# jin-s13/GKGNet

Measured on AMD Instinct MI355X. Metric: Grapher fwd+bwd images/sec, higher is better.
Workload: dtype f32; 1 GPU; BASELINE cfg2-literal: Grapher(C320,G4,k9,d1,18x18,relpos)+GrapherLabel(L80) fwd+bwd; batch_per_gpu=32, global_batch=32, C=320, G=4, HW=18x18, k=9, dilation=1, bn=local, parallelism=dp1, input_layout=nchw, launch=hipGraph replay of fwd+bwd+grad-pack, world_size=1, backend=none (single process), grad_allreduce=none (1 GPU)

## Files before the change

### gkgnet_amd/csrc/gkg_dense.hip

```cpp
#include "gkg_common.h"

namespace gkg {

template <typename OutT, bool STATS = false>
__global__ __launch_bounds__(256) void nchw_to_tm_kernel(const float* __restrict__ x, OutT* __restrict__ out,
                                                         int C, int N, const float* __restrict__ img_scale,
                                                         const float* __restrict__ add_tm = nullptr,
                                                         const float* __restrict__ y = nullptr, const float* __restrict__ mean = nullptr,
                                                         const float* __restrict__ invstd = nullptr, double* __restrict__ asums = nullptr) {
  constexpr int TS = STATS ? 4 : 1;
  __shared__ float tile[TS][32][33];
  const int b = blockIdx.z, c0 = blockIdx.y * 32, n0 = blockIdx.x * 32 * TS;
  const int tx = threadIdx.x & 31, ty = threadIdx.x >> 5;
#pragma unroll
  for (int s = 0; s < TS; ++s)
#pragma unroll
    for (int i = 0; i < 4; ++i) {
      const int ch = c0 + ty + 8 * i, n = n0 + 32 * s + tx;
      tile[s][ty + 8 * i][tx] = (ch < C && n < N) ? x[((size_t)b * C + ch) * N + n] : 0.f;
    }
  const float sc = img_scale ? img_scale[b] : 1.0f;
  float mv = 0.f, iv = 0.f, s0 = 0.f, s1 = 0.f;
  float av[TS][4], yv[TS][4];
  if constexpr (STATS) {
// ... 284 lines not shown
    const float* p = part + (size_t)q * nblk * C2 + (ln >> 2) * C + ch;
    int b = ln & 3;
    for (; b + 28 < nblk; b += 32) {
      float v[8];
#pragma unroll
      for (int u = 0; u < 8; ++u) v[u] = p[(size_t)(b + 4 * u) * C2];
#pragma unroll
      for (int u = 0; u < 8; ++u) acc += (double)v[u];
    }
    for (; b < nblk; b += 4) acc += (double)p[(size_t)b * C2];
  }
  lane_sum[ln][t] = acc;
  __syncthreads();
  if (ln != 0 || ch >= C) return;
  const double S = (lane_sum[0][t] + lane_sum[1][t]) + (lane_sum[2][t] + lane_sum[3][t]);
  const double Q = (lane_sum[4][t] + lane_sum[5][t]) + (lane_sum[6][t] + lane_sum[7][t]);
  const size_t o = (size_t)q * C + ch;
  const double ms = S / R;
  double var = Q / R - ms * ms;
  if (var < 0.0) var = 0.0;
  const double m = ms + (y_shift_row ? (double)y_shift_row[(size_t)q * R * C + ch] : 0.0);
  const float is = (float)(1.0 / sqrt(var + (double)eps));
  const float av = gamma[o] * is;
  a[o] = av;
  cs[o] = (float)((double)beta[o] - (double)av * m);
  mean[o] = (float)m;
  invstd[o] = is;
  if (running_mean) {
    const float bv = bias ? bias[o] : 0.f;
    running_mean[o] = (1.f - momentum) * running_mean[o] + momentum * ((float)m + bv);
    const double unb = R > 1 ? var * (double)R / (double)(R - 1) : var;
    running_var[o] = (1.f - momentum) * running_var[o] + momentum * (float)unb;
  }
}

__global__ void bn_finalize_kernel(const float* __restrict__ sums, const float* __restrict__ gamma,
                                   const float* __restrict__ beta, const float* __restrict__ bias,
                                   float* __restrict__ running_mean, float* __restrict__ running_var,
                                   float* __restrict__ a, float* __restrict__ cs, float* __restrict__ mean,
                                   float* __restrict__ invstd, const float* __restrict__ count, int C, float momentum,
                                   float eps, long long* __restrict__ num_batches_tracked) {
  const int ch = blockIdx.x * blockDim.x + threadIdx.x;
  if (num_batches_tracked && ch == 0 && blockIdx.y == 0) *num_batches_tracked += 1;
  if (ch >= C) return;
  const double R = (double)count[0];
  const int q = blockIdx.y;
  sums += (size_t)q * 2 * C; gamma += (size_t)q * C; beta += (size_t)q * C; a += (size_t)q * C; cs += (size_t)q * C;
  mean += (size_t)q * C; invstd += (size_t)q * C;
  if (bias) bias += (size_t)q * C;
  if (running_mean) { running_mean += (size_t)q * C; running_var += (size_t)q * C; }
  const double m = (double)sums[ch] / R;
  double var = (double)sums[C + ch] / R - m * m;
  if (var < 0.0) var = 0.0;
  const float is = (float)(1.0 / sqrt(var + (double)eps));
  const float av = gamma[ch] * is;
  a[ch] = av;
  cs[ch] = beta[ch] - av * (float)m;
  mean[ch] = (float)m;
  invstd[ch] = is;
  if (running_mean) {
    const float b = bias ? bias[ch] : 0.f;
    running_mean[ch] = (1.f - momentum) * running_mean[ch] + momentum * ((float)m + b);
    const double unb = R > 1.0 ? var * R / (R - 1.0) : var;
    running_var[ch] = (1.f - momentum) * running_var[ch] + momentum * (float)unb;
  }
}

__global__ void bn_eval_affine_kernel(const float* __restrict__ gamma, const float* __restrict__ beta,
                                      const float* __restrict__ bias, const float* __restrict__ running_mean,
                                      const float* __restrict__ running_var, float* __restrict__ a,
                                      float* __restrict__ cs, int C, float eps) {
  const int ch = blockIdx.x * blockDim.x + threadIdx.x;
  if (ch >= C) return;
  const float av = gamma[ch] / sqrtf(running_var[ch] + eps);
  a[ch] = av;
  cs[ch] = beta[ch] + av * ((bias ? bias[ch] : 0.f) - running_mean[ch]);
}

template <int ACT, typename OutT>
__global__ __launch_bounds__(256) void affine_act_kernel(const float* __restrict__ y, const float* __restrict__ a,
                                                         const float* __restrict__ cs, const float* __restrict__ res,
                                                         OutT* __restrict__ out, size_t total4, int C, int ldo,
                                                         size_t o_bstride, const float* __restrict__ row_scale,
                                                         int rows_per_scale, uint16_t* __restrict__ out2, BnDerive d,
                                                         int ochunk = 0) {
  extern __shared__ float ac_tab[];
  const int C4 = C >> 2;
  const int q = blockIdx.y;
  y += (size_t)q * total4 * 4; out += (size_t)q * o_bstride;
  if (res) res += (size_t)q * total4 * 4;
  if (d.sums) {
    const bool side = blockIdx.x == 0;
    for (int ch = threadIdx.x; ch < C; ch += 256) {
      float av, cv;
      bn_derive_channel(d, (size_t)q * C + ch, d.sums[(size_t)q * 2 * C + ch], d.sums[(size_t)q * 2 * C + C + ch], side, av, cv);
      ac_tab[ch] = av; ac_tab[C + ch] = cv;
    }
    if (side && q == 0) {
      if (threadIdx.x == 0 && d.nbt) *d.nbt += 1;
      for (size_t i = threadIdx.x; i < d.zero_doubles; i += 256) d.zero_buf[i] = 0.0;
    }
    __syncthreads();
    a = ac_tab; cs = ac_tab + C;
  } else {
    a += (size_t)q * C; cs += (size_t)q * C;
  }
  for (size_t i = (size_t)blockIdx.x * 256 + threadIdx.x; i < total4; i += (size_t)gridDim.x * 256) {
    const size_t r = i / C4;
    const int cg = (int)(i - r * C4);
    const float4 v = *reinterpret_cast<const float4*>(y + 4 * i);
    const float4 a4 = *reinterpret_cast<const float4*>(a + 4 * cg);
    const float4 c4 = *reinterpret_cast<const float4*>(cs + 4 * cg);
    float4 o;
    o.x = __builtin_fmaf(a4.x, v.x, c4.x); o.y = __builtin_fmaf(a4.y, v.y, c4.y);
    o.z = __builtin_fmaf(a4.z, v.z, c4.z); o.w = __builtin_fmaf(a4.w, v.w, c4.w);
    if (ACT == 1) { o.x = gelu_f(o.x); o.y = gelu_f(o.y); o.z = gelu_f(o.z); o.w = gelu_f(o.w); }
    if (row_scale) {
      const float sc = row_scale[r / rows_per_scale];
      o.x *= sc; o.y *= sc; o.z *= sc; o.w *= sc;
    }
    if (res) {
      const float4 rv = *reinterpret_cast<const float4*>(res + 4 * i);
      o.x += rv.x; o.y += rv.y; o.z += rv.z; o.w += rv.w;
    }
    const int oc = ochunk > 0 ? 4 * cg + (4 * cg / ochunk) * ochunk : 4 * cg;
    stf4(out + r * (size_t)ldo + oc, o);
    if (out2) stf4(out2 + r * (size_t)ldo + oc, o);
  }
}

template <int ACT>
__global__ __launch_bounds__(256) void affine_act_bf16in_kernel(const uint16_t* __restrict__ y, const float* __restrict__ a,
                                                                const float* __restrict__ cs, float* __restrict__ out32,
                                                                uint16_t* __restrict__ out16, size_t total8, int C) {
  const int C8 = C >> 3;
  for (size_t i = (size_t)blockIdx.x * 256 + threadIdx.x; i < total8; i += (size_t)gridDim.x * 256) {
    const int cg = (int)(i % C8);
    const uint4 v = *reinterpret_cast<const uint4*>(y + 8 * i);
    const uint32_t w[4] = {v.x, v.y, v.z, v.w};
    float o[8];
#pragma unroll
    for (int u = 0; u < 4; ++u) {
      o[2 * u] = __uint_as_float(w[u] << 16);
      o[2 * u + 1] = __uint_as_float(w[u] & 0xffff0000u);
    }
#pragma unroll
    for (int u = 0; u < 8; ++u) {
      o[u] = __builtin_fmaf(a[8 * cg + u], o[u], cs[8 * cg + u]);
      if (ACT == 1) o[u] = gelu_f(o[u]);
    }
    if (out32) {
      stf4(out32 + 8 * i, make_float4(o[0], o[1], o[2], o[3]));
      stf4(out32 + 8 * i + 4, make_float4(o[4], o[5], o[6], o[7]));
    }
    if (out16)
      *reinterpret_cast<uint4*>(out16 + 8 * i) = make_uint4(pack_bf16x2(o[0], o[1]), pack_bf16x2(o[2], o[3]),
                                                             pack_bf16x2(o[4], o[5]), pack_bf16x2(o[6], o[7]));
  }
}

template <int ACT>
__global__ __launch_bounds__(256) void bn_bwd_apply_d_kernel(const float* dout, const float* __restrict__ y,
                                                             const float* __restrict__ a, const float* __restrict__ cs,
                                                             const float* __restrict__ mean, const float* __restrict__ invstd,
                                                             const double* __restrict__ dsums, float* dy,
                                                             size_t total4, int C, int R, int ldg, size_t g_bstride,
                                                             float* __restrict__ dgamma, float* __restrict__ dbeta,
                                                             double* __restrict__ zero_buf, size_t zero_doubles,
                                                             const float* __restrict__ row_scale = nullptr, int rows_per_scale = 1,
                                                             const double* __restrict__ gsums = nullptr,
                                                             const float* __restrict__ count = nullptr) {
  const int C4 = C >> 2;
  const float invR = 1.0f / (count ? count[0] : (float)R);
  const int q = blockIdx.y;
  y += (size_t)q * total4 * 4; dy += (size_t)q * total4 * 4; dout += (size_t)q * g_bstride;
  a += (size_t)q * C; cs += (size_t)q * C; mean += (size_t)q * C; invstd += (size_t)q * C; dsums += (size_t)q * 2 * C;
  if (blockIdx.x == 0) {
    for (int ch = threadIdx.x; ch < C; ch += 256) {
      dbeta[(size_t)q * C + ch] = (float)dsums[ch];
      dgamma[(size_t)q * C + ch] = (float)dsums[C + ch];
    }
    if (q == 0)
      for (size_t i = threadIdx.x; i < zero_doubles; i += 256) zero_buf[i] = 0.0;
  }
  if (gsums) dsums = gsums + (size_t)q * 2 * C;
  for (size_t i = (size_t)blockIdx.x * 256 + threadIdx.x; i < total4; i += (size_t)gridDim.x * 256) {
    const size_t r = i / C4;
    const int cg = (int)(i - r * C4);
    const float4 g = *reinterpret_cast<const float4*>(dout + r * (size_t)ldg + 4 * cg);
    const float4 v = *reinterpret_cast<const float4*>(y + 4 * i);
    const float4 a4 = *reinterpret_cast<const float4*>(a + 4 * cg);
    const float4 c4 = *reinterpret_cast<const float4*>(cs + 4 * cg);
    const float4 m4 = *reinterpret_cast<const float4*>(mean + 4 * cg);
    const float4 i4 = *reinterpret_cast<const float4*>(invstd + 4 * cg);
    const double2 sa = *reinterpret_cast<const double2*>(dsums + 4 * cg), sb = *reinterpret_cast<const double2*>(dsums + 4 * cg + 2);
    const double2 qa = *reinterpret_cast<const double2*>(dsums + C + 4 * cg), qb = *reinterpret_cast<const double2*>(dsums + C + 4 * cg + 2);
    const float4 s4 = make_float4((float)sa.x, (float)sa.y, (float)sb.x, (float)sb.y);
    const float4 q4 = make_float4((float)qa.x, (float)qa.y, (float)qb.x, (float)qb.y);
    float4 dz = g;
    if (row_scale) {
      const float sc = row_scale[r / (size_t)rows_per_scale];
      dz.x *= sc; dz.y *= sc; dz.z *= sc; dz.w *= sc;
    }
    if (ACT == 1) {
      dz.x *= gelu_grad_f(__builtin_fmaf(a4.x, v.x, c4.x)); dz.y *= gelu_grad_f(__builtin_fmaf(a4.y, v.y, c4.y));
      dz.z *= gelu_grad_f(__builtin_fmaf(a4.z, v.z, c4.z)); dz.w *= gelu_grad_f(__builtin_fmaf(a4.w, v.w, c4.w));
    }
    float4 o;
    o.x = a4.x * (dz.x - s4.x * invR - ((v.x - m4.x) * i4.x) * (q4.x * invR));
    o.y = a4.y * (dz.y - s4.y * invR - ((v.y - m4.y) * i4.y) * (q4.y * invR));
// ... 86 lines not shown
#pragma unroll 4
    for (int r = r0 + rl; r < r1; r += ST_RL) {
      const float4 g = *reinterpret_cast<const float4*>(dout + (size_t)r * ldg + 4 * cgi);
      const float4 v = *reinterpret_cast<const float4*>(y + (size_t)r * C + 4 * cgi);
      float4 dz = g;
      if (row_scale) {
        const float sc = row_scale[r / rows_per_scale];
        dz.x *= sc; dz.y *= sc; dz.z *= sc; dz.w *= sc;
      }
      if (ACT == 1) {
        dz.x *= gelu_grad_f(__builtin_fmaf(a4.x, v.x, c4.x)); dz.y *= gelu_grad_f(__builtin_fmaf(a4.y, v.y, c4.y));
        dz.z *= gelu_grad_f(__builtin_fmaf(a4.z, v.z, c4.z)); dz.w *= gelu_grad_f(__builtin_fmaf(a4.w, v.w, c4.w));
      }
      *reinterpret_cast<float4*>(dy + (size_t)r * C + 4 * cgi) = make_float4(a4.x * dz.x, a4.y * dz.y, a4.z * dz.z, a4.w * dz.w);
      s[0] += (double)dz.x; s[1] += (double)dz.y; s[2] += (double)dz.z; s[3] += (double)dz.w;
      sq[0] += (double)dz.x * (double)v.x; sq[1] += (double)dz.y * (double)v.y;
      sq[2] += (double)dz.z * (double)v.z; sq[3] += (double)dz.w * (double)v.w;
    }
  }
#pragma unroll
  for (int j = 0; j < 4; ++j) { red[0][rl][4 * cg + j] = s[j]; red[1][rl][4 * cg + j] = sq[j]; }
  __syncthreads();
  if (tid < 8 * ST_CG) {
    const int which = tid >> 6, col = tid & 63;
    double acc = 0.0;
#pragma unroll
    for (int l = 0; l < ST_RL; ++l) acc += red[which][l][col];
    const int ch = blockIdx.y * 4 * ST_CG + col;
    if (ch < C) {
      if (asums) __hip_atomic_fetch_add(asums + ((size_t)q * 2 + which) * C + ch, acc, __ATOMIC_RELAXED, __HIP_MEMORY_SCOPE_AGENT);
      else part[(((size_t)q * gridDim.x + blockIdx.x) * 2 + which) * C + ch] = (float)acc;
    }
  }
}

__global__ __launch_bounds__(256) void bn_eval_bwd_finish_kernel(const double* __restrict__ dsums, const float* __restrict__ part,
                                                                 int nblk, const float* __restrict__ a,
                                                                 const float* __restrict__ running_mean,
                                                                 const float* __restrict__ running_var,
                                                                 const float* __restrict__ bias, float eps, int C,
                                                                 float* __restrict__ dgamma, float* __restrict__ dbeta,
                                                                 float* __restrict__ dbias, double* __restrict__ zero_buf,
                                                                 size_t zero_doubles) {
  const int q = blockIdx.y;
  if (blockIdx.x == 0 && q == 0)
    for (size_t i = threadIdx.x; i < zero_doubles; i += 256) zero_buf[i] = 0.0;
  const int ch = blockIdx.x * 256 + threadIdx.x;
  if (ch >= C) return;
  double S0 = 0.0, S1 = 0.0;
  if (dsums) {
    S0 = dsums[(size_t)q * 2 * C + ch];
    S1 = dsums[(size_t)q * 2 * C + C + ch];
  } else {
    const float* p = part + (size_t)q * nblk * 2 * C + ch;
    for (int b = 0; b < nblk; ++b) { S0 += (double)p[(size_t)b * 2 * C]; S1 += (double)p[(size_t)b * 2 * C + C]; }
  }
  const size_t o = (size_t)q * C + ch;
  if (dbeta) dbeta[o] = (float)S0;
  if (dgamma) {
    const double sh = (bias ? (double)bias[o] : 0.0) - (double)running_mean[o];
    dgamma[o] = (float)((S1 + sh * S0) / sqrt((double)running_var[o] + (double)eps));
  }
  if (dbias) dbias[o] = (float)((double)a[o] * S0);
}

}

using namespace gkg;

static int stats_tiles(int C) { return ((C >> 2) + ST_CG - 1) / ST_CG; }

static int stats_blocks(int R, int C, int nb, int* rows_per_block) {
  const int cols = stats_tiles(C) * nb;
  int nblk = (768 + cols - 1) / cols;
  const int cap = cols >= 4 ? 128 : 256;
  if (nblk > cap) nblk = cap;
  const int by_rows = (R + ST_RL - 1) / ST_RL;
  if (nblk > by_rows) nblk = by_rows;
  if (nblk < 1) nblk = 1;
  *rows_per_block = (R + nblk - 1) / nblk;
  return (R + *rows_per_block - 1) / *rows_per_block;
}

static bool bad_c(int C) { return C <= 0 || (C & 3) != 0 || C > 4096; }

extern "C" size_t gkg_bn_workspace_bytes(int R, int C, int nb) {
  if (R <= 0 || bad_c(C) || nb <= 0) return 0;
  int rpb;
  const int nblk = stats_blocks(R, C, nb, &rpb);
  return (size_t)nb * (nblk + 1) * 2 * C * sizeof(float);
}

extern "C" int gkg_nchw_to_tm(const float* x, void* out, int B, int C, int N, int out_dtype, const float* img_scale,
                              void* stream) {
  if (!x || !out) return gkg_fail(GKG_ERR_NULL, "gkg_nchw_to_tm: null pointer");
  if (B <= 0 || C <= 0 || N <= 0 || B > 65535) return gkg_fail(GKG_ERR_SHAPE, "gkg_nchw_to_tm: bad sizes");
  if (out_dtype != GKG_F32 && out_dtype != GKG_BF16) return gkg_fail(GKG_ERR_UNSUPPORTED, "gkg_nchw_to_tm: out_dtype is GKG_F32 or GKG_BF16");
  dim3 grid((N + 31) / 32, (C + 31) / 32, B);
  if (out_dtype == GKG_BF16) hipLaunchKernelGGL(nchw_to_tm_kernel<uint16_t>, grid, dim3(256), 0, (hipStream_t)stream, x, (uint16_t*)out, C, N, img_scale);
  else hipLaunchKernelGGL(nchw_to_tm_kernel<float>, grid, dim3(256), 0, (hipStream_t)stream, x, (float*)out, C, N, img_scale);
  hipError_t e = hipGetLastError();
  return e == hipSuccess ? 0 : gkg_fail_hip(e, "nchw_to_tm_kernel");
}

extern "C" int gkg_nchw_to_tm_add(const float* x, const float* add_tm, float* out, int B, int C, int N, void* stream) {
  if (!x || !add_tm || !out) return gkg_fail(GKG_ERR_NULL, "gkg_nchw_to_tm_add: null pointer");
  if (B <= 0 || C <= 0 || N <= 0 || B > 65535) return gkg_fail(GKG_ERR_SHAPE, "gkg_nchw_to_tm_add: bad sizes");
  dim3 grid((N + 31) / 32, (C + 31) / 32, B);
  hipLaunchKernelGGL(nchw_to_tm_kernel<float>, grid, dim3(256), 0, (hipStream_t)stream, x, out, C, N, (const float*)nullptr, add_tm);
  hipError_t e = hipGetLastError();
  return e == hipSuccess ? 0 : gkg_fail_hip(e, "nchw_to_tm_kernel (add)");
}

extern "C" int gkg_nchw_to_tm_add_bnstats(const float* x, const float* add_tm, float* out, const float* y, const float* mean,
                                          const float* invstd, double* sums, int B, int C, int N, void* stream) {
  if (!x || !out || !y || !mean || !invstd || !sums) return gkg_fail(GKG_ERR_NULL, "gkg_nchw_to_tm_add_bnstats: null pointer");
  if (B <= 0 || C <= 0 || N <= 0 || B > 65535) return gkg_fail(GKG_ERR_SHAPE, "gkg_nchw_to_tm_add_bnstats: bad sizes");
  dim3 grid((N + 127) / 128, (C + 31) / 32, B);
  hipLaunchKernelGGL((nchw_to_tm_kernel<float, true>), grid, dim3(256), 0, (hipStream_t)stream, x, out, C, N, (const float*)nullptr, add_tm,
                     y, mean, invstd, sums);
  hipError_t e = hipGetLastError();
  return e == hipSuccess ? 0 : gkg_fail_hip(e, "nchw_to_tm_kernel (add + BN backward statistics)");
}

extern "C" int gkg_tm_affine_to_nchw_dual(const float* y, const float* a, const float* c, const float* res_tm, float* out,
                                          float* out_tm, int B, int C, int N, void* stream) {
  if (!y || !out || !res_tm || !out_tm || ((a == nullptr) != (c == nullptr))) return gkg_fail(GKG_ERR_NULL, "gkg_tm_affine_to_nchw_dual: null pointer");
  if (B <= 0 || C <= 0 || N <= 0 || B > 65535) return gkg_fail(GKG_ERR_SHAPE, "gkg_tm_affine_to_nchw_dual: bad sizes");
  dim3 grid((N + 31) / 32, (C + 31) / 32, B);
  hipLaunchKernelGGL(tm_affine_to_nchw_kernel, grid, dim3(256), 0, (hipStream_t)stream, y, a, c, (const float*)nullptr, out, C, N,
                     (const float*)nullptr, BnDerive{}, res_tm, out_tm);
  hipError_t e = hipGetLastError();
  return e == hipSuccess ? 0 : gkg_fail_hip(e, "tm_affine_to_nchw_kernel (dual)");
}

extern "C" int gkg_tm_affine_to_nchw(const float* y, const float* a, const float* c, const float* res, float* out,
                                     int B, int C, int N, const float* img_scale, void* stream) {
  if (!y || !out || ((a == nullptr) != (c == nullptr))) return gkg_fail(GKG_ERR_NULL, "gkg_tm_affine_to_nchw: null pointer");
  if (B <= 0 || C <= 0 || N <= 0 || B > 65535) return gkg_fail(GKG_ERR_SHAPE, "gkg_tm_affine_to_nchw: bad sizes");
  dim3 grid((N + 31) / 32, (C + 31) / 32, B);
  hipLaunchKernelGGL(tm_affine_to_nchw_kernel, grid, dim3(256), 0, (hipStream_t)stream, y, a, c, res, out, C, N, img_scale, BnDerive{});
  hipError_t e = hipGetLastError();
  return e == hipSuccess ? 0 : gkg_fail_hip(e, "tm_affine_to_nchw_kernel");
}

extern "C" int gkg_bn_train_stats(const float* y, const float* gamma, const float* beta, const float* bias,
                                  float* running_mean, float* running_var, float* a, float* c, float* mean,
                                  float* invstd, int R, int C, int nb, float momentum, float eps,
                                  long long* num_batches_tracked, void* workspace, size_t workspace_bytes, void* stream) {
  if (!y || !gamma || !beta || !a || !c || !mean || !invstd || !workspace)
    return gkg_fail(GKG_ERR_NULL, "gkg_bn_train_stats: null pointer");
  if (R <= 0 || bad_c(C) || nb <= 0 || nb > 64) return gkg_fail(GKG_ERR_SHAPE, "gkg_bn_train_stats: need R > 0, C % 4 == 0, C <= 4096, 1 <= nb <= 64");
  if ((running_mean == nullptr) != (running_var == nullptr)) return gkg_fail(GKG_ERR_NULL, "gkg_bn_train_stats: running stats come in pairs");
  int rpb;
  const int nblk = stats_blocks(R, C, nb, &rpb);
  if (workspace_bytes < (size_t)nb * (nblk + 1) * 2 * C * sizeof(float))
    return gkg_fail(GKG_ERR_WORKSPACE, "gkg_bn_train_stats: workspace too small (gkg_bn_workspace_bytes)");
  hipStream_t st = (hipStream_t)stream;
  float* part = (float*)workspace;
  float* sums = part + (size_t)nb * nblk * 2 * C;
  hipLaunchKernelGGL(col_stats_kernel<true>, dim3(nblk, stats_tiles(C), nb), dim3(256), 0, st, y, part, R, C, rpb);
  hipLaunchKernelGGL(reduce_finalize_kernel, dim3((C + 31) / 32, nb), dim3(256), 0, st, part, nblk, gamma, beta, bias,
                     running_mean, running_var, a, c, mean, invstd, R, C, momentum, eps, num_batches_tracked, y);
  hipError_t e = hipGetLastError();
  return e == hipSuccess ? 0 : gkg_fail_hip(e, "bn_train_stats");
}

extern "C" int gkg_bn_eval_affine(const float* gamma, const float* beta, const float* bias, const float* running_mean,
                                  const float* running_var, float* a, float* c, int C, float eps, void* stream) {
  if (!gamma || !beta || !running_mean || !running_var || !a || !c) return gkg_fail(GKG_ERR_NULL, "gkg_bn_eval_affine: null pointer");
  if (C <= 0) return gkg_fail(GKG_ERR_SHAPE, "gkg_bn_eval_affine: bad C");
  hipLaunchKernelGGL(bn_eval_affine_kernel, dim3((C + 255) / 256), dim3(256), 0, (hipStream_t)stream, gamma, beta, bias,
                     running_mean, running_var, a, c, C, eps);
  hipError_t e = hipGetLastError();
  return e == hipSuccess ? 0 : gkg_fail_hip(e, "bn_eval_affine_kernel");
}

extern "C" int gkg_avgpool_tm(const float* x, int ldx, int xchunk, float* out, int B, int H, int W, int C, int r, void* stream) {
  if (!x || !out) return gkg_fail(GKG_ERR_NULL, "gkg_avgpool_tm: null pointer");
  if (ldx == 0) ldx = C;
  if (B <= 0 || H <= 0 || W <= 0 || bad_c(C) || r <= 0 || H / r <= 0 || W / r <= 0 || ldx < C || (ldx & 3) || xchunk < 0 || (xchunk & 3) ||
      (xchunk > 0 && (C % xchunk || ldx < 2 * C)) || ((size_t)x & 15) || ((size_t)out & 15))
    return gkg_fail(GKG_ERR_SHAPE, "gkg_avgpool_tm: bad sizes (C % 4 == 0, r <= H, W; 16-byte aligned rows)");
  const size_t total4 = (size_t)B * (H / r) * (W / r) * (C >> 2);
  if ((total4 + 255) / 256 > 0x7fffffffull) return gkg_fail(GKG_ERR_UNSUPPORTED, "gkg_avgpool_tm: too large for one launch");
  hipLaunchKernelGGL(avgpool_tm_kernel, dim3((unsigned)((total4 + 255) / 256)), dim3(256), 0, (hipStream_t)stream, x, out, H, W, C, r, ldx,
                     xchunk, total4);
  hipError_t e = hipGetLastError();
  return e == hipSuccess ? 0 : gkg_fail_hip(e, "avgpool_tm_kernel");
}

extern "C" int gkg_affine_act(const float* y, const float* a, const float* c, const float* res, void* out, int R, int C,
                              int nb, int ldo, size_t out_bstride, int ochunk, int act, int out_dtype, const float* row_scale,
                              int rows_per_scale, void* stream) {
  if (row_scale && rows_per_scale <= 0) return gkg_fail(GKG_ERR_SHAPE, "gkg_affine_act: rows_per_scale must be positive");
  if (ochunk < 0 || (ochunk & 3) || (ochunk > 0 && (C % ochunk || ldo < 2 * C)))
    return gkg_fail(GKG_ERR_SHAPE, "gkg_affine_act: ochunk must be a multiple of 4 dividing C, with ldo >= 2 C");
  if (!y || !a || !c || !out) return gkg_fail(GKG_ERR_NULL, "gkg_affine_act: null pointer");
  if (R <= 0 || bad_c(C) || nb <= 0 || nb > 64 || ldo < C || (ldo & 3) || (out_bstride & 3) || (act != 0 && act != 1))
    return gkg_fail(GKG_ERR_SHAPE, "gkg_affine_act: bad sizes");
  if (out_dtype != GKG_F32 && out_dtype != GKG_BF16) return gkg_fail(GKG_ERR_UNSUPPORTED, "gkg_affine_act: out_dtype is GKG_F32 or GKG_BF16");
  const size_t total4 = (size_t)R * (C >> 2);
  const int blocks = (int)((total4 + 255) / 256 > 2048 ? 2048 : (total4 + 255) / 256);
  const dim3 grid(blocks, nb);
  hipStream_t st = (hipStream_t)stream;
  if (out_dtype == GKG_BF16) {
    uint16_t* o = (uint16_t*)out;
    if (act == 1) hipLaunchKernelGGL((affine_act_kernel<1, uint16_t>), grid, dim3(256), 0, st, y, a, c, res, o, total4, C, ldo, out_bstride, row_scale, rows_per_scale, (uint16_t*)nullptr, BnDerive{}, ochunk);
    else hipLaunchKernelGGL((affine_act_kernel<0, uint16_t>), grid, dim3(256), 0, st, y, a, c, res, o, total4, C, ldo, out_bstride, row_scale, rows_per_scale, (uint16_t*)nullptr, BnDerive{}, ochunk);
  } else {
    float* o = (float*)out;
    if (act == 1) hipLaunchKernelGGL((affine_act_kernel<1, float>), grid, dim3(256), 0, st, y, a, c, res, o, total4, C, ldo, out_bstride, row_scale, rows_per_scale, (uint16_t*)nullptr, BnDerive{}, ochunk);
    else hipLaunchKernelGGL((affine_act_kernel<0, float>), grid, dim3(256), 0, st, y, a, c, res, o, total4, C, ldo, out_bstride, row_scale, rows_per_scale, (uint16_t*)nullptr, BnDerive{}, ochunk);
  }
  hipError_t e = hipGetLastError();
  return e == hipSuccess ? 0 : gkg_fail_hip(e, "affine_act_kernel");
}

extern "C" int gkg_affine_act_bf16in(const void* y_bf16, const float* a, const float* c, float* out_f32, void* out_bf16, int R,
                                     int C, int act, void* stream) {
  if (!y_bf16 || !a || !c || (!out_f32 && !out_bf16)) return gkg_fail(GKG_ERR_NULL, "gkg_affine_act_bf16in: null pointer");
  if (R <= 0 || C <= 0 || (C & 7) || (act != 0 && act != 1)) return gkg_fail(GKG_ERR_SHAPE, "gkg_affine_act_bf16in: bad sizes (C % 8 == 0)");
  const size_t total8 = (size_t)R * (C >> 3);
  const int blocks = (int)((total8 + 255) / 256 > 4096 ? 4096 : (total8 + 255) / 256);
  hipStream_t st = (hipStream_t)stream;
  if (act == 1) hipLaunchKernelGGL((affine_act_bf16in_kernel<1>), dim3(blocks), dim3(256), 0, st, (const uint16_t*)y_bf16, a, c, out_f32, (uint16_t*)out_bf16, total8, C);
  else hipLaunchKernelGGL((affine_act_bf16in_kernel<0>), dim3(blocks), dim3(256), 0, st, (const uint16_t*)y_bf16, a, c, out_f32, (uint16_t*)out_bf16, total8, C);
  hipError_t e = hipGetLastError();
  return e == hipSuccess ? 0 : gkg_fail_hip(e, "affine_act_bf16in_kernel");
}

extern "C" int gkg_affine_act_dual(const float* y, const float* a, const float* c, const float* res, float* out_f32,
                                   void* out_bf16, int R, int C, int act, const float* row_scale, int rows_per_scale,
                                   void* stream) {
  if (row_scale && rows_per_scale <= 0) return gkg_fail(GKG_ERR_SHAPE, "gkg_affine_act_dual: rows_per_scale must be positive");
  if (!y || !a || !c || !out_f32 || !out_bf16) return gkg_fail(GKG_ERR_NULL, "gkg_affine_act_dual: null pointer");
  if (R <= 0 || bad_c(C) || (act != 0 && act != 1)) return gkg_fail(GKG_ERR_SHAPE, "gkg_affine_act_dual: bad sizes");
  const size_t total4 = (size_t)R * (C >> 2);
  const int blocks = (int)((total4 + 255) / 256 > 2048 ? 2048 : (total4 + 255) / 256);
  hipStream_t st = (hipStream_t)stream;
  if (act == 1) hipLaunchKernelGGL((affine_act_kernel<1, float>), dim3(blocks, 1), dim3(256), 0, st, y, a, c, res, out_f32, total4, C, C, (size_t)0, row_scale, rows_per_scale, (uint16_t*)out_bf16, BnDerive{});
  else hipLaunchKernelGGL((affine_act_kernel<0, float>), dim3(blocks, 1), dim3(256), 0, st, y, a, c, res, out_f32, total4, C, C, (size_t)0, row_scale, rows_per_scale, (uint16_t*)out_bf16, BnDerive{});
  hipError_t e = hipGetLastError();
  return e == hipSuccess ? 0 : gkg_fail_hip(e, "affine_act_kernel (dual)");
}

extern "C" int gkg_bn_bwd(const float* dout, const float* y, const float* a, const float* c, const float* mean,
                          const float* invstd, float* dy, float* dgamma, float* dbeta, int R, int C, int nb, int ldg,
                          size_t dout_bstride, int act, void* workspace, size_t workspace_bytes, void* stream) {
  if (!dout || !y || !a || !c || !mean || !invstd || !dy || !dgamma || !dbeta || !workspace)
    return gkg_fail(GKG_ERR_NULL, "gkg_bn_bwd: null pointer");
  if (R <= 0 || bad_c(C) || nb <= 0 || nb > 64 || ldg < C || (ldg & 3) || (dout_bstride & 3) || (act != 0 && act != 1))
    return gkg_fail(GKG_ERR_SHAPE, "gkg_bn_bwd: bad sizes");
  int rpb;
  const int nblk = stats_blocks(R, C, nb, &rpb);
  if (workspace_bytes < (size_t)nb * (nblk + 1) * 2 * C * sizeof(float)) return gkg_fail(GKG_ERR_WORKSPACE, "gkg_bn_bwd: workspace too small");
  hipStream_t st = (hipStream_t)stream;
  float* part = (float*)workspace;
  float* sums = part + (size_t)nb * nblk * 2 * C;
  if (act == 1) hipLaunchKernelGGL((bn_bwd_stats_kernel<1>), dim3(nblk, stats_tiles(C), nb), dim3(256), 0, st, dout, y, a, c, mean, invstd, part, R, C, rpb, ldg, dout_bstride, (float*)nullptr);
  else hipLaunchKernelGGL((bn_bwd_stats_kernel<0>), dim3(nblk, stats_tiles(C), nb), dim3(256), 0, st, dout, y, a, c, mean, invstd, part, R, C, rpb, ldg, dout_bstride, (float*)nullptr);
  hipLaunchKernelGGL(reduce_partials_kernel, dim3((2 * C + 31) / 32, nb), dim3(256), 0, st, part, sums, nblk, 2 * C, dbeta, dgamma);
  const size_t total4 = (size_t)R * (C >> 2);
  const int blocks = (int)((total4 + 255) / 256 > 2048 ? 2048 : (total4 + 255) / 256);
  if (act == 1) hipLaunchKernelGGL((bn_bwd_apply_kernel<1>), dim3(blocks, nb), dim3(256), 0, st, dout, y, a, c, mean, invstd, sums, dy, total4, C, R, ldg, dout_bstride, (const float*)nullptr);
  else hipLaunchKernelGGL((bn_bwd_apply_kernel<0>), dim3(blocks, nb), dim3(256), 0, st, dout, y, a, c, mean, invstd, sums, dy, total4, C, R, ldg, dout_bstride, (const float*)nullptr);
  hipError_t e = hipGetLastError();
  return e == hipSuccess ? 0 : gkg_fail_hip(e, "bn_bwd");
}

static int bn_bwd_atomic_impl(const float* dout, const float* y, const float* a, const float* c, const float* mean,
                              const float* invstd, float* dy, float* dgamma, float* dbeta, int R, int C, int nb, int ldg,
                              size_t dout_bstride, int act, double* sums, double* zero_buf, size_t zero_doubles, void* stream,
                              bool stats_pass, const float* row_scale = nullptr, int rows_per_scale = 1, bool apply_pass = true,
                              const double* gsums = nullptr, const float* count = nullptr);

extern "C" int gkg_bn_bwd_atomic(const float* dout, const float* y, const float* a, const float* c, const float* mean,
                                 const float* invstd, float* dy, float* dgamma, float* dbeta, int R, int C, int nb, int ldg,
                                 size_t dout_bstride, int act, double* sums, double* zero_buf, size_t zero_doubles, void* stream) {
  if (!dout || !y || !a || !c || !mean || !invstd || !dy || !dgamma || !dbeta || !sums)
    return gkg_fail(GKG_ERR_NULL, "gkg_bn_bwd_atomic: null pointer");
  if (R <= 0 || bad_c(C) || nb <= 0 || nb > 64 || ldg < C || (ldg & 3) || (dout_bstride & 3) || (act != 0 && act != 1) ||
      (zero_doubles && !zero_buf))
    return gkg_fail(GKG_ERR_SHAPE, "gkg_bn_bwd_atomic: bad sizes");
  return bn_bwd_atomic_impl(dout, y, a, c, mean, invstd, dy, dgamma, dbeta, R, C, nb, ldg, dout_bstride, act, sums, zero_buf,
                            zero_doubles, stream, true);
}

extern "C" int gkg_bn_bwd_atomic_scaled(const float* dout, const float* y, const float* a, const float* c, const float* mean,
                                        const float* invstd, float* dy, float* dgamma, float* dbeta, int R, int C, int nb,
                                        int ldg, size_t dout_bstride, int act, double* sums, double* zero_buf,
                                        size_t zero_doubles, const float* row_scale, int rows_per_scale, void* stream) {
  if (!dout || !y || !a || !c || !mean || !invstd || !dy || !dgamma || !dbeta || !sums || !row_scale)
    return gkg_fail(GKG_ERR_NULL, "gkg_bn_bwd_atomic_scaled: null pointer");
  if (R <= 0 || bad_c(C) || nb <= 0 || nb > 64 || ldg < C || (ldg & 3) || (dout_bstride & 3) || (act != 0 && act != 1) ||
      (zero_doubles && !zero_buf) || rows_per_scale <= 0)
    return gkg_fail(GKG_ERR_SHAPE, "gkg_bn_bwd_atomic_scaled: bad sizes");
  return bn_bwd_atomic_impl(dout, y, a, c, mean, invstd, dy, dgamma, dbeta, R, C, nb, ldg, dout_bstride, act, sums, zero_buf,
                            zero_doubles, stream, true, row_scale, rows_per_scale);
}

extern "C" int gkg_bn_bwd_apply_from_sums(const float* dout, const float* y, const float* a, const float* c, const float* mean,
                                          const float* invstd, float* dy, float* dgamma, float* dbeta, int R, int C, int nb,
                                          int ldg, size_t dout_bstride, int act, const double* sums, double* zero_buf,
                                          size_t zero_doubles, void* stream) {
  if (!dout || !y || !a || !c || !mean || !invstd || !dy || !dgamma || !dbeta || !sums)
    return gkg_fail(GKG_ERR_NULL, "gkg_bn_bwd_apply_from_sums: null pointer");
  if (R <= 0 || bad_c(C) || nb <= 0 || nb > 64 || ldg < C || (ldg & 3) || (dout_bstride & 3) || (act != 0 && act != 1) ||
      (zero_doubles && !zero_buf))
    return gkg_fail(GKG_ERR_SHAPE, "gkg_bn_bwd_apply_from_sums: bad sizes");
  return bn_bwd_atomic_impl(dout, y, a, c, mean, invstd, dy, dgamma, dbeta, R, C, nb, ldg, dout_bstride, act,
                            const_cast<double*>(sums), zero_buf, zero_doubles, stream, false);
}

extern "C" int gkg_bn_eval_bwd(const float* dout, const float* y, const float* a, const float* c, float* dy, int R, int C, int nb,
                               int ldg, size_t dout_bstride, int act, const float* row_scale, int rows_per_scale,
                               const float* running_mean, const float* running_var, const float* bias, float eps, float* dgamma,
                               float* dbeta, float* dbias, double* sums, double* zero_buf, size_t zero_doubles, void* workspace,
                               size_t workspace_bytes, void* stream) {
  if (!dout || !y || !a || !c || !dy) return gkg_fail(GKG_ERR_NULL, "gkg_bn_eval_bwd: null pointer");
  if (R <= 0 || bad_c(C) || nb <= 0 || nb > 64 || ldg < C || (ldg & 3) || (dout_bstride & 3) || (act != 0 && act != 1) ||
      (zero_doubles && !zero_buf) || (row_scale && rows_per_scale <= 0))
    return gkg_fail(GKG_ERR_SHAPE, "gkg_bn_eval_bwd: bad sizes");
  const bool want = dgamma || dbeta || dbias;
  if (dgamma && (!running_mean || !running_var)) return gkg_fail(GKG_ERR_NULL, "gkg_bn_eval_bwd: dgamma needs the running statistics");
// ... 15 lines not shown
  else { if (act == 1) GKG_EVAL_BWD(1, false); else GKG_EVAL_BWD(0, false); }
#undef GKG_EVAL_BWD
  if (want)
    hipLaunchKernelGGL(bn_eval_bwd_finish_kernel, dim3((C + 255) / 256, nb), dim3(256), 0, st, (const double*)sums, (const float*)part, nblk,
                       a, running_mean, running_var, bias, eps, C, dgamma, dbeta, dbias, zero_buf, zero_doubles);
  hipError_t e = hipGetLastError();
  return e == hipSuccess ? 0 : gkg_fail_hip(e, "bn_eval_bwd");
}


static int bn_bwd_atomic_impl(const float* dout, const float* y, const float* a, const float* c, const float* mean,
                              const float* invstd, float* dy, float* dgamma, float* dbeta, int R, int C, int nb, int ldg,
                              size_t dout_bstride, int act, double* sums, double* zero_buf, size_t zero_doubles, void* stream,
                              bool stats_pass, const float* row_scale, int rows_per_scale, bool apply_pass, const double* gsums,
                              const float* count) {
  int rpb;
  const int nblk = stats_blocks(R, C, nb, &rpb);
  hipStream_t st = (hipStream_t)stream;
  if (stats_pass) {
    if (act == 1) hipLaunchKernelGGL((bn_bwd_stats_kernel<1>), dim3(nblk, stats_tiles(C), nb), dim3(256), 0, st, dout, y, a, c, mean, invstd, (float*)nullptr, R, C, rpb, ldg, dout_bstride, (float*)nullptr, sums, row_scale, rows_per_scale);
    else hipLaunchKernelGGL((bn_bwd_stats_kernel<0>), dim3(nblk, stats_tiles(C), nb), dim3(256), 0, st, dout, y, a, c, mean, invstd, (float*)nullptr, R, C, rpb, ldg, dout_bstride, (float*)nullptr, sums, row_scale, rows_per_scale);
  }
  if (apply_pass) {
    const size_t total4 = (size_t)R * (C >> 2);
    const int blocks = (int)((total4 + 255) / 256 > 2048 ? 2048 : (total4 + 255) / 256);
    if (act == 1) hipLaunchKernelGGL((bn_bwd_apply_d_kernel<1>), dim3(blocks, nb), dim3(256), 0, st, dout, y, a, c, mean, invstd, sums, dy, total4, C, R, ldg, dout_bstride, dgamma, dbeta, zero_buf, zero_doubles, row_scale, rows_per_scale, gsums, count);
    else hipLaunchKernelGGL((bn_bwd_apply_d_kernel<0>), dim3(blocks, nb), dim3(256), 0, st, dout, y, a, c, mean, invstd, sums, dy, total4, C, R, ldg, dout_bstride, dgamma, dbeta, zero_buf, zero_doubles, row_scale, rows_per_scale, gsums, count);
  }
  hipError_t e = hipGetLastError();
  return e == hipSuccess ? 0 : gkg_fail_hip(e, "bn_bwd_atomic");
}

extern "C" int gkg_bn_bwd_stats_f64(const float* dout, const float* y, const float* a, const float* c, const float* mean,
                                    const float* invstd, int R, int C, int nb, int ldg, size_t dout_bstride, int act, double* sums,
                                    const float* row_scale, int rows_per_scale, void* stream) {
  if (!dout || !y || !a || !c || !mean || !invstd || !sums) return gkg_fail(GKG_ERR_NULL, "gkg_bn_bwd_stats_f64: null pointer");
  if (R <= 0 || bad_c(C) || nb <= 0 || nb > 64 || ldg < C || (ldg & 3) || (dout_bstride & 3) || (act != 0 && act != 1) ||
      (row_scale && rows_per_scale <= 0))
    return gkg_fail(GKG_ERR_SHAPE, "gkg_bn_bwd_stats_f64: bad sizes");
  return bn_bwd_atomic_impl(dout, y, a, c, mean, invstd, nullptr, nullptr, nullptr, R, C, nb, ldg, dout_bstride, act, sums, nullptr, 0,
                            stream, true, row_scale, row_scale ? rows_per_scale : 1, false);
}

extern "C" int gkg_bn_bwd_apply_sync(const float* dout, const float* y, const float* a, const float* c, const float* mean,
                                     const float* invstd, float* dy, float* dgamma, float* dbeta, int R, int C, int nb, int ldg,
                                     size_t dout_bstride, int act, const double* sums_local, const double* sums_global,
                                     const float* count, double* zero_buf, size_t zero_doubles, const float* row_scale,
                                     int rows_per_scale, void* stream) {
  if (!dout || !y || !a || !c || !mean || !invstd || !dy || !dgamma || !dbeta || !sums_local || !sums_global || !count)
    return gkg_fail(GKG_ERR_NULL, "gkg_bn_bwd_apply_sync: null pointer");
  if (R <= 0 || bad_c(C) || nb <= 0 || nb > 64 || ldg < C || (ldg & 3) || (dout_bstride & 3) || (act != 0 && act != 1) ||
      (zero_doubles && !zero_buf) || (row_scale && rows_per_scale <= 0) || (((size_t)sums_local | (size_t)sums_global) & 15))
    return gkg_fail(GKG_ERR_SHAPE, "gkg_bn_bwd_apply_sync: bad sizes");
  return bn_bwd_atomic_impl(dout, y, a, c, mean, invstd, dy, dgamma, dbeta, R, C, nb, ldg, dout_bstride, act,
                            const_cast<double*>(sums_local), zero_buf, zero_doubles, stream, false, row_scale,
                            row_scale ? rows_per_scale : 1, true, sums_global, count);
}

static int bn_apply_train_impl(const float* y, const double* sums, const float* gamma, const float* beta, const float* bias,
                               float* running_mean, float* running_var, long long* num_batches_tracked, float* a, float* c,
                               float* mean, float* invstd, const float* res, float* out, int R, int C, int nb, int ldo,
                               size_t out_bstride, int ochunk, int act, int nchw_B, const float* row_scale, int rows_per_scale,
                               float momentum, float eps, double* zero_buf, size_t zero_doubles, void* stream,
                               const double* count, float* count_out) {
  if (!y || !sums || !gamma || !beta || !a || !c || !mean || !invstd || !out)
    return gkg_fail(GKG_ERR_NULL, "gkg_bn_apply_train: null pointer");
  if ((running_mean == nullptr) != (running_var == nullptr)) return gkg_fail(GKG_ERR_NULL, "gkg_bn_apply_train: running stats come in pairs");
  if (R <= 0 || bad_c(C) || nb <= 0 || nb > 64 || (act != 0 && act != 1) || (zero_doubles && !zero_buf) || nchw_B < 0)
    return gkg_fail(GKG_ERR_SHAPE, "gkg_bn_apply_train: bad sizes");
  BnDerive d{sums, gamma, beta, bias, running_mean, running_var, num_batches_tracked, a, c, mean, invstd, R, momentum, eps,
             zero_buf, zero_doubles, count, count_out};
  hipStream_t st = (hipStream_t)stream;
  if (nchw_B > 0) {
    if (nb != 1 || act != 0 || R % nchw_B) return gkg_fail(GKG_ERR_SHAPE, "gkg_bn_apply_train: channel-major output needs nb == 1, act == 0, R % B == 0");
    const int N = R / nchw_B;
    dim3 grid((N + 31) / 32, (C + 31) / 32, nchw_B);
    hipLaunchKernelGGL(tm_affine_to_nchw_kernel, grid, dim3(256), 0, st, y, (const float*)nullptr, (const float*)nullptr, res, out, C, N,
                       row_scale, d);
  } else {
    if (row_scale && rows_per_scale <= 0) return gkg_fail(GKG_ERR_SHAPE, "gkg_bn_apply_train: rows_per_scale must be positive");
    if (ldo < C || (ldo & 3) || (out_bstride & 3)) return gkg_fail(GKG_ERR_SHAPE, "gkg_bn_apply_train: bad output pitch");
    if (ochunk < 0 || (ochunk & 3) || (ochunk > 0 && (C % ochunk || ldo < 2 * C)))
      return gkg_fail(GKG_ERR_SHAPE, "gkg_bn_apply_train: ochunk must be a multiple of 4 dividing C, with ldo >= 2 C");
    const size_t total4 = (size_t)R * (C >> 2);
    const int blocks = (int)((total4 + 255) / 256 > 2048 ? 2048 : (total4 + 255) / 256);
    const dim3 grid(blocks, nb);
    const size_t lds = (size_t)2 * C * sizeof(float);
    if (act == 1) hipLaunchKernelGGL((affine_act_kernel<1, float>), grid, dim3(256), lds, st, y, (const float*)nullptr, (const float*)nullptr, res, out, total4, C, ldo, out_bstride, row_scale, rows_per_scale, (uint16_t*)nullptr, d, ochunk);
    else hipLaunchKernelGGL((affine_act_kernel<0, float>), grid, dim3(256), lds, st, y, (const float*)nullptr, (const float*)nullptr, res, out, total4, C, ldo, out_bstride, row_scale, rows_per_scale, (uint16_t*)nullptr, d, ochunk);
  }
  hipError_t e = hipGetLastError();
  return e == hipSuccess ? 0 : gkg_fail_hip(e, "bn_apply_train");
}

extern "C" int gkg_bn_apply_train(const float* y, const double* sums, const float* gamma, const float* beta, const float* bias,
                                  float* running_mean, float* running_var, long long* num_batches_tracked, float* a, float* c,
                                  float* mean, float* invstd, const float* res, float* out, int R, int C, int nb, int ldo,
                                  size_t out_bstride, int ochunk, int act, int nchw_B, const float* row_scale, int rows_per_scale,
                                  float momentum, float eps, double* zero_buf, size_t zero_doubles, void* stream) {
  return bn_apply_train_impl(y, sums, gamma, beta, bias, running_mean, running_var, num_batches_tracked, a, c, mean, invstd, res, out,
                             R, C, nb, ldo, out_bstride, ochunk, act, nchw_B, row_scale, rows_per_scale, momentum, eps, zero_buf,
                             zero_doubles, stream, nullptr, nullptr);
}

extern "C" int gkg_bn_apply_train_sync(const float* y, const double* sums, const float* gamma, const float* beta, const float* bias,
                                       float* running_mean, float* running_var, long long* num_batches_tracked, float* a, float* c,
                                       float* mean, float* invstd, const float* res, float* out, int R, int C, int nb, int ldo,
                                       size_t out_bstride, int ochunk, int act, int nchw_B, const float* row_scale,
                                       int rows_per_scale, float momentum, float eps, double* zero_buf, size_t zero_doubles,
                                       const double* count, float* count_out, void* stream) {
  if (!count) return gkg_fail(GKG_ERR_NULL, "gkg_bn_apply_train_sync: null count");
  return bn_apply_train_impl(y, sums, gamma, beta, bias, running_mean, running_var, num_batches_tracked, a, c, mean, invstd, res, out,
                             R, C, nb, ldo, out_bstride, ochunk, act, nchw_B, row_scale, rows_per_scale, momentum, eps, zero_buf,
                             zero_doubles, stream, count, count_out);
}

static int bn_apply_train_dual_impl(const float* y, const double* sums, const float* gamma, const float* beta, const float* bias,
                                    float* running_mean, float* running_var, long long* num_batches_tracked, float* a,
                                    float* c, float* mean, float* invstd, const float* res_tm, float* out, float* out_tm,
                                    int B, int C, int N, float momentum, float eps, double* zero_buf, size_t zero_doubles,
                                    void* stream, const double* count, float* count_out) {
  if (!y || !sums || !gamma || !beta || !a || !c || !mean || !invstd || !out || !res_tm || !out_tm)
    return gkg_fail(GKG_ERR_NULL, "gkg_bn_apply_train_dual: null pointer");
  if ((running_mean == nullptr) != (running_var == nullptr)) return gkg_fail(GKG_ERR_NULL, "gkg_bn_apply_train_dual: running stats come in pairs");
  if (B <= 0 || B > 65535 || N <= 0 || bad_c(C) || (zero_doubles && !zero_buf)) return gkg_fail(GKG_ERR_SHAPE, "gkg_bn_apply_train_dual: bad sizes");
  BnDerive d{sums, gamma, beta, bias, running_mean, running_var, num_batches_tracked, a, c, mean, invstd, B * N, momentum, eps,
             zero_buf, zero_doubles, count, count_out};
  dim3 grid((N + 31) / 32, (C + 31) / 32, B);
  hipLaunchKernelGGL(tm_affine_to_nchw_kernel, grid, dim3(256), 0, (hipStream_t)stream, y, (const float*)nullptr, (const float*)nullptr,
                     (const float*)nullptr, out, C, N, (const float*)nullptr, d, res_tm, out_tm);
  hipError_t e = hipGetLastError();
  return e == hipSuccess ? 0 : gkg_fail_hip(e, "bn_apply_train (dual)");
}

extern "C" int gkg_bn_apply_train_dual(const float* y, const double* sums, const float* gamma, const float* beta, const float* bias,
                                       float* running_mean, float* running_var, long long* num_batches_tracked, float* a,
                                       float* c, float* mean, float* invstd, const float* res_tm, float* out, float* out_tm,
                                       int B, int C, int N, float momentum, float eps, double* zero_buf, size_t zero_doubles,
                                       void* stream) {
  return bn_apply_train_dual_impl(y, sums, gamma, beta, bias, running_mean, running_var, num_batches_tracked, a, c, mean, invstd,
                                  res_tm, out, out_tm, B, C, N, momentum, eps, zero_buf, zero_doubles, stream, nullptr, nullptr);
}

extern "C" int gkg_bn_apply_train_dual_sync(const float* y, const double* sums, const float* gamma, const float* beta,
                                            const float* bias, float* running_mean, float* running_var,
                                            long long* num_batches_tracked, float* a, float* c, float* mean, float* invstd,
                                            const float* res_tm, float* out, float* out_tm, int B, int C, int N, float momentum,
                                            float eps, double* zero_buf, size_t zero_doubles, const double* count, float* count_out,
                                            void* stream) {
  if (!count) return gkg_fail(GKG_ERR_NULL, "gkg_bn_apply_train_dual_sync: null count");
  return bn_apply_train_dual_impl(y, sums, gamma, beta, bias, running_mean, running_var, num_batches_tracked, a, c, mean, invstd,
                                  res_tm, out, out_tm, B, C, N, momentum, eps, zero_buf, zero_doubles, stream, count, count_out);
}

extern "C" int gkg_bn_stats_sums(const float* y, float* sums, int R, int C, int nb, void* workspace,
                                 size_t workspace_bytes, void* stream) {
  if (!y || !sums || !workspace) return gkg_fail(GKG_ERR_NULL, "gkg_bn_stats_sums: null pointer");
  if (R <= 0 || bad_c(C) || nb <= 0 || nb > 64) return gkg_fail(GKG_ERR_SHAPE, "gkg_bn_stats_sums: bad sizes");
  int rpb;
  const int nblk = stats_blocks(R, C, nb, &rpb);
  if (workspace_bytes < (size_t)nb * (nblk + 1) * 2 * C * sizeof(float))
    return gkg_fail(GKG_ERR_WORKSPACE, "gkg_bn_stats_sums: workspace too small (gkg_bn_workspace_bytes)");
  hipStream_t st = (hipStream_t)stream;
  float* part = (float*)workspace;
  hipLaunchKernelGGL(col_stats_kernel<false>, dim3(nblk, stats_tiles(C), nb), dim3(256), 0, st, y, part, R, C, rpb);
  hipLaunchKernelGGL(reduce_partials_kernel, dim3((2 * C + 31) / 32, nb), dim3(256), 0, st, part, sums, nblk, 2 * C,
                     (float*)nullptr, (float*)nullptr);
  hipError_t e = hipGetLastError();
  return e == hipSuccess ? 0 : gkg_fail_hip(e, "bn_stats_sums");
}

extern "C" int gkg_bn_finalize(const float* sums, const float* count, const float* gamma, const float* beta,
// ... 47 lines not shown
```

Baseline: 41220 images/s.

## Tile BN train-apply by channel slice so each block derives only its channels

Replaces the grid-stride BN apply used in training with a 2D-tiled kernel. Each block now covers a column slice of channels and a row range, so it derives scale and shift only for its own channels instead of every block recomputing all C channels from double sums. Loads of the first rows are issued before the derive step, and rows are prefetched in groups of four. This adds more template variants and a heuristic for tile and block counts.

```diff
diff --git a/gkgnet_amd/csrc/gkg_dense.hip b/gkgnet_amd/csrc/gkg_dense.hip
--- a/gkgnet_amd/csrc/gkg_dense.hip
+++ b/gkgnet_amd/csrc/gkg_dense.hip
@@ -390,29 +390,12 @@
                                                          const float* __restrict__ cs, const float* __restrict__ res,
                                                          OutT* __restrict__ out, size_t total4, int C, int ldo,
                                                          size_t o_bstride, const float* __restrict__ row_scale,
-                                                         int rows_per_scale, uint16_t* __restrict__ out2, BnDerive d,
-                                                         int ochunk = 0) {
-  extern __shared__ float ac_tab[];
+                                                         int rows_per_scale, uint16_t* __restrict__ out2, int ochunk = 0) {
   const int C4 = C >> 2;
   const int q = blockIdx.y;
   y += (size_t)q * total4 * 4; out += (size_t)q * o_bstride;
   if (res) res += (size_t)q * total4 * 4;
-  if (d.sums) {
-    const bool side = blockIdx.x == 0;
-    for (int ch = threadIdx.x; ch < C; ch += 256) {
-      float av, cv;
-      bn_derive_channel(d, (size_t)q * C + ch, d.sums[(size_t)q * 2 * C + ch], d.sums[(size_t)q * 2 * C + C + ch], side, av, cv);
-      ac_tab[ch] = av; ac_tab[C + ch] = cv;
-    }
-    if (side && q == 0) {
-      if (threadIdx.x == 0 && d.nbt) *d.nbt += 1;
-      for (size_t i = threadIdx.x; i < d.zero_doubles; i += 256) d.zero_buf[i] = 0.0;
-    }
-    __syncthreads();
-    a = ac_tab; cs = ac_tab + C;
-  } else {
-    a += (size_t)q * C; cs += (size_t)q * C;
-  }
+  a += (size_t)q * C; cs += (size_t)q * C;
   for (size_t i = (size_t)blockIdx.x * 256 + threadIdx.x; i < total4; i += (size_t)gridDim.x * 256) {
     const size_t r = i / C4;
     const int cg = (int)(i - r * C4);
@@ -434,6 +417,74 @@
     const int oc = ochunk > 0 ? 4 * cg + (4 * cg / ochunk) * ochunk : 4 * cg;
     stf4(out + r * (size_t)ldo + oc, o);
     if (out2) stf4(out2 + r * (size_t)ldo + oc, o);
+  }
+}
+
+constexpr int AP_PF = 4;
+template <int ACT, bool RES>
+__global__ __launch_bounds__(256) void bn_apply_tiled_kernel(const float* __restrict__ y, const float* __restrict__ res,
+                                                             float* __restrict__ out, int R, int C, int ldo, size_t o_bstride,
+                                                             const float* __restrict__ row_scale, int rows_per_scale, BnDerive d,
+                                                             int ochunk, int tile4, int rows_per_block) {
+  __shared__ float ac_tab[2][256];
+  const int tid = threadIdx.x;
+  const int q = blockIdx.z;
+  const int C4 = C >> 2;
+  const int RL = 256 / tile4;
+  const int rl = tid / tile4;
+  const int cg = tid - rl * tile4;
+  const int cgi = blockIdx.y * tile4 + cg;
+  const int r1 = (int)min((long long)R, ((long long)blockIdx.x + 1) * rows_per_block);
+  y += (size_t)q * R * C + 4 * min(cgi, C4 - 1); out += (size_t)q * o_bstride;
+  if (RES) res += (size_t)q * R * C + 4 * min(cgi, C4 - 1);
+  int r = (rl < RL && cgi < C4) ? (int)blockIdx.x * rows_per_block + rl : r1;
+  const int chd = blockIdx.y * 4 * tile4 + tid;
+  const bool derive = tid < 4 * tile4 && chd < C;
+  double S = 0.0, Q = 0.0;
+  if (derive) { S = d.sums[(size_t)q * 2 * C + chd]; Q = d.sums[(size_t)q * 2 * C + C + chd]; }
+  float4 v[AP_PF], rv[AP_PF];
+  float sc[AP_PF];
+  auto request = [&]() __attribute__((always_inline)) {
+#pragma unroll
+    for (int u = 0; u < AP_PF; ++u) {
+      const int ru = min(r + u * RL, r1 - 1);
+      v[u] = *reinterpret_cast<const float4*>(y + (size_t)ru * C);
+      if (RES) rv[u] = *reinterpret_cast<const float4*>(res + (size_t)ru * C);
+      if (row_scale) sc[u] = row_scale[ru / rows_per_scale];
+    }
+  };
+  request();
+  if (derive) {
+    float av, cv;
+    bn_derive_channel(d, (size_t)q * C + chd, S, Q, blockIdx.x == 0, av, cv);
+    ac_tab[0][tid] = av; ac_tab[1][tid] = cv;
+  }
+  if (blockIdx.x == 0 && blockIdx.y == 0 && q == 0) {
+    if (tid == 0 && d.nbt) *d.nbt += 1;
+    for (size_t i = tid; i < d.zero_doubles; i += 256) d.zero_buf[i] = 0.0;
+  }
+  __syncthreads();
+  if (r >= r1) return;
+  const float4 a4 = *reinterpret_cast<const float4*>(&ac_tab[0][4 * cg]);
+  const float4 c4 = *reinterpret_cast<const float4*>(&ac_tab[1][4 * cg]);
+  out += ochunk > 0 ? 4 * cgi + (4 * cgi / ochunk) * ochunk : 4 * cgi;
+  for (;;) {
+#pragma unroll
+    for (int u = 0; u < AP_PF; ++u) {
+      const int ru = r + u * RL;
+      if (ru < r1) {
+        float4 o;
+        o.x = __builtin_fmaf(a4.x, v[u].x, c4.x); o.y = __builtin_fmaf(a4.y, v[u].y, c4.y);
+        o.z = __builtin_fmaf(a4.z, v[u].z, c4.z); o.w = __builtin_fmaf(a4.w, v[u].w, c4.w);
+        if (ACT == 1) { o.x = gelu_f(o.x); o.y = gelu_f(o.y); o.z = gelu_f(o.z); o.w = gelu_f(o.w); }
+        if (row_scale) { o.x *= sc[u]; o.y *= sc[u]; o.z *= sc[u]; o.w *= sc[u]; }
+        if (RES) { o.x += rv[u].x; o.y += rv[u].y; o.z += rv[u].z; o.w += rv[u].w; }
+        stf4(out + (size_t)ru * ldo, o);
+      }
+    }
+    r += AP_PF * RL;
+    if (r >= r1) break;
+    request();
   }
 }
 
@@ -686,6 +737,19 @@
   return (R + *rows_per_block - 1) / *rows_per_block;
 }
 
+static int apply_blocks(int R, int C, int nb, int act, int* tile4, int* rows_per_block) {
+  const int C4 = C >> 2;
+  const int tiles = (C4 + 63) / 64;
+  *tile4 = (C4 & 15) == 0 ? 16 : (C4 + tiles - 1) / tiles;
+  const int min_rows = (act == 1 ? 1 : AP_PF) * (256 / *tile4);
+  const int cols = ((C4 + *tile4 - 1) / *tile4) * nb;
+  long long nblk = (1024 + cols - 1) / cols;
+  const long long by_rows = ((long long)R + min_rows - 1) / min_rows;
+  if (nblk > by_rows) nblk = by_rows;
+  *rows_per_block = (int)((R + nblk - 1) / nblk);
+  return (int)((R + (long long)*rows_per_block - 1) / *rows_per_block);
+}
+
 static bool bad_c(int C) { return C <= 0 || (C & 3) != 0 || C > 4096; }
 
 extern "C" size_t gkg_bn_workspace_bytes(int R, int C, int nb) {
@@ -810,12 +874,12 @@
   hipStream_t st = (hipStream_t)stream;
   if (out_dtype == GKG_BF16) {
     uint16_t* o = (uint16_t*)out;
-    if (act == 1) hipLaunchKernelGGL((affine_act_kernel<1, uint16_t>), grid, dim3(256), 0, st, y, a, c, res, o, total4, C, ldo, out_bstride, row_scale, rows_per_scale, (uint16_t*)nullptr, BnDerive{}, ochunk);
-    else hipLaunchKernelGGL((affine_act_kernel<0, uint16_t>), grid, dim3(256), 0, st, y, a, c, res, o, total4, C, ldo, out_bstride, row_scale, rows_per_scale, (uint16_t*)nullptr, BnDerive{}, ochunk);
+    if (act == 1) hipLaunchKernelGGL((affine_act_kernel<1, uint16_t>), grid, dim3(256), 0, st, y, a, c, res, o, total4, C, ldo, out_bstride, row_scale, rows_per_scale, (uint16_t*)nullptr, ochunk);
+    else hipLaunchKernelGGL((affine_act_kernel<0, uint16_t>), grid, dim3(256), 0, st, y, a, c, res, o, total4, C, ldo, out_bstride, row_scale, rows_per_scale, (uint16_t*)nullptr, ochunk);
   } else {
     float* o = (float*)out;
-    if (act == 1) hipLaunchKernelGGL((affine_act_kernel<1, float>), grid, dim3(256), 0, st, y, a, c, res, o, total4, C, ldo, out_bstride, row_scale, rows_per_scale, (uint16_t*)nullptr, BnDerive{}, ochunk);
-    else hipLaunchKernelGGL((affine_act_kernel<0, float>), grid, dim3(256), 0, st, y, a, c, res, o, total4, C, ldo, out_bstride, row_scale, rows_per_scale, (uint16_t*)nullptr, BnDerive{}, ochunk);
+    if (act == 1) hipLaunchKernelGGL((affine_act_kernel<1, float>), grid, dim3(256), 0, st, y, a, c, res, o, total4, C, ldo, out_bstride, row_scale, rows_per_scale, (uint16_t*)nullptr, ochunk);
+    else hipLaunchKernelGGL((affine_act_kernel<0, float>), grid, dim3(256), 0, st, y, a, c, res, o, total4, C, ldo, out_bstride, row_scale, rows_per_scale, (uint16_t*)nullptr, ochunk);
   }
   hipError_t e = hipGetLastError();
   return e == hipSuccess ? 0 : gkg_fail_hip(e, "affine_act_kernel");
@@ -843,8 +907,8 @@
   const size_t total4 = (size_t)R * (C >> 2);
   const int blocks = (int)((total4 + 255) / 256 > 2048 ? 2048 : (total4 + 255) / 256);
   hipStream_t st = (hipStream_t)stream;
-  if (act == 1) hipLaunchKernelGGL((affine_act_kernel<1, float>), dim3(blocks, 1), dim3(256), 0, st, y, a, c, res, out_f32, total4, C, C, (size_t)0, row_scale, rows_per_scale, (uint16_t*)out_bf16, BnDerive{});
-  else hipLaunchKernelGGL((affine_act_kernel<0, float>), dim3(blocks, 1), dim3(256), 0, st, y, a, c, res, out_f32, total4, C, C, (size_t)0, row_scale, rows_per_scale, (uint16_t*)out_bf16, BnDerive{});
+  if (act == 1) hipLaunchKernelGGL((affine_act_kernel<1, float>), dim3(blocks, 1), dim3(256), 0, st, y, a, c, res, out_f32, total4, C, C, (size_t)0, row_scale, rows_per_scale, (uint16_t*)out_bf16);
+  else hipLaunchKernelGGL((affine_act_kernel<0, float>), dim3(blocks, 1), dim3(256), 0, st, y, a, c, res, out_f32, total4, C, C, (size_t)0, row_scale, rows_per_scale, (uint16_t*)out_bf16);
   hipError_t e = hipGetLastError();
   return e == hipSuccess ? 0 : gkg_fail_hip(e, "affine_act_kernel (dual)");
 }
@@ -1026,12 +1090,12 @@
     if (ldo < C || (ldo & 3) || (out_bstride & 3)) return gkg_fail(GKG_ERR_SHAPE, "gkg_bn_apply_train: bad output pitch");
     if (ochunk < 0 || (ochunk & 3) || (ochunk > 0 && (C % ochunk || ldo < 2 * C)))
       return gkg_fail(GKG_ERR_SHAPE, "gkg_bn_apply_train: ochunk must be a multiple of 4 dividing C, with ldo >= 2 C");
-    const size_t total4 = (size_t)R * (C >> 2);
-    const int blocks = (int)((total4 + 255) / 256 > 2048 ? 2048 : (total4 + 255) / 256);
-    const dim3 grid(blocks, nb);
-    const size_t lds = (size_t)2 * C * sizeof(float);
-    if (act == 1) hipLaunchKernelGGL((affine_act_kernel<1, float>), grid, dim3(256), lds, st, y, (const float*)nullptr, (const float*)nullptr, res, out, total4, C, ldo, out_bstride, row_scale, rows_per_scale, (uint16_t*)nullptr, d, ochunk);
-    else hipLaunchKernelGGL((affine_act_kernel<0, float>), grid, dim3(256), lds, st, y, (const float*)nullptr, (const float*)nullptr, res, out, total4, C, ldo, out_bstride, row_scale, rows_per_scale, (uint16_t*)nullptr, d, ochunk);
+    if (R > 0x7fffffff - 4 * 256 * AP_PF) return gkg_fail(GKG_ERR_UNSUPPORTED, "gkg_bn_apply_train: too many rows for one launch");
+    int tile4, rpb;
+    const dim3 grid(apply_blocks(R, C, nb, act, &tile4, &rpb), ((C >> 2) + tile4 - 1) / tile4, nb);
+    auto kern = act == 1 ? (res ? bn_apply_tiled_kernel<1, true> : bn_apply_tiled_kernel<1, false>)
+                         : (res ? bn_apply_tiled_kernel<0, true> : bn_apply_tiled_kernel<0, false>);
+    hipLaunchKernelGGL(kern, grid, dim3(256), 0, st, y, res, out, R, C, ldo, out_bstride, row_scale, rows_per_scale, d, ochunk, tile4, rpb);
   }
   hipError_t e = hipGetLastError();
   return e == hipSuccess ? 0 : gkg_fail_hip(e, "bn_apply_train");
```

After: 41710 images/s (median of 6 runs). +1.2%, better.
